# gridap/GridapSolvers.jl

Hardware: AMD Instinct MI355X
Metric: DoFs/sec, CG+GMG V-cycle on 3D Poisson Q1 (higher is better)
Workload: dtype f64; 1 GPU; BASELINE configs[1]: 3D Poisson Q1 128^3 cells, 4-level GMG V-cycle, Richardson(Jacobi,10,2/3) pre=post, dense-inverse coarse solve, CG rtol=1e-06, rhs=u=x1+x2 Dirichlet lift; dofs=2048383, nnz=54439939, levels=4

## Files before the change

### gridapsolvers.jl_amd/csrc/gmg_amd.hip

```cpp
#include "../../include/gmg_amd.h"
#include "kernels.hpp"
#include "comm.hpp"

#include <algorithm>
#include <cmath>
#include <cstdarg>
#include <cstdio>
#include <cstdlib>
#include <cstring>
#include <functional>
#include <map>
#include <memory>
#include <mutex>
#include <exception>
#include <string>
#include <thread>
#include <atomic>
#include <chrono>
#include <unordered_map>
#include <vector>

using namespace gmg;

namespace {
// ... 346 lines not shown
  DevCSR A, P, R;
  double *dinv = nullptr;
  Smoother pre, post;
  Smoother pcorr;
  bool has_pcorr = false;
  HostCSR hG;
  bool hasG = false;
  DevCSR G;
  double *ptmp = nullptr, *pcor = nullptr;
  bool post_shares_pre = true;
  int64_t n = 0;
  int64_t nvec = 0;
  HaloPlan halo;
  bool split = false;
  struct HostXfer { struct ::gmg_solver *solver; int level; } hostctx{nullptr, 0};
  int64_t nbnd = 0;
  int32_t *gh_rows = nullptr;
  int64_t *gh_ptr = nullptr;
  int32_t *gh_col = nullptr;
  double *gh_val = nullptr;
  int32_t *gh_len = nullptr, *gh_scol = nullptr;
  int64_t *gh_soff = nullptr;
  double *gh_sval = nullptr;
  uint8_t *gh_scode = nullptr;
  double *gh_dict = nullptr;
  bool r_split = false;
  GhostFix rfix;
  double *x = nullptr;
  double *rbuf[2] = {nullptr, nullptr};
  double *sbuf[2] = {nullptr, nullptr};
  uint32_t *pflags = nullptr;
  int pf_nwg = 0;
  uint32_t pf_epoch = 1;
  double *dx = nullptr;
  double *rcur = nullptr;
};

struct ConvLog {
  int maxiter = 0;
  double atol = 0, rtol = 0;
  int num_iters = 0;
  std::vector<double> residuals;
  void configure(int mi, double a, double r)
  {
    maxiter = mi; atol = a; rtol = r;
    residuals.assign((size_t)std::max(mi, 0) + 1, 0.0);
  }
  bool finished(int niter, double e_a, double e_r) const
  {
    return (niter >= maxiter) || (e_r < rtol) || (e_a < atol);
  }
  bool init(double r0)
  {
    num_iters = 0;
    std::fill(residuals.begin(), residuals.end(), 0.0);
    residuals[0] = r0;
    return finished(num_iters, r0, 1.0);
  }
  bool update(double r)
  {
    num_iters += 1;
    if ((size_t)num_iters < residuals.size()) residuals[num_iters] = r;
    return finished(num_iters, r, r / residuals[0]);
  }
  int finalize(double r) const
  {
// ... 186 lines not shown
  int sell_un = 6;
  int nt_loads = 1;
  int nt_rowwise = 1;
  int xcd_remap_big = -1;
  int64_t big_rows = 4000000;
  int sell_defer = 1;
  bool big_level(const DevCSR &M) const { return M.nrows > big_rows; }
  int remap_for_big(const DevCSR &M, int rows_per_wg, int nwg) const
  {
    if (xcd_remap_big >= 0) return xcd_remap_big == 1 ? xcd_remap : xcd_remap_big;
    const int64_t want = (2 * std::max<int64_t>(M.band, 1) + rows_per_wg - 1) / rows_per_wg;
    if (want < 2 || want * 8 * 4 > nwg) return 0;
    return (int)want;
  }
  int use_pattern = 1;
  int pat_un = 9;
  int pat_wgs = 2048;
  int pat_rb = 3;
  int use_opattern = 1;
  int pat_batched = 1;
  int pat_nb = 0;
  int pat_small_wpb = 4;
  int pat_small_wpb2 = 2;
  int pat_emit = 1;
  int64_t pat_coded_min_rows = 500000;
  int gj_mfma = 1;
  int pat_tile = 0;
  int64_t pat_tile_rows = 3500000;
  int pat_wide = 1;
  int pat_strict = 1;
  int persist_wpb_min = 1;
  int persist = 1;
  int persist_regs = 1;
  int persist_fenced = 0;
  int persist_max_slices = 0;
  int n_cus = 0;
  uint32_t *d_perr_dev = nullptr;
  uint32_t *h_perr = nullptr, *d_perr = nullptr;
  int pat_bcast = 1;
  int pat_r2 = 1;
  int pat_zwalk = 1;
  int64_t pat_zwalk_wide_rows = 1000000;
  int pat_zwalk_wide = 1;
  int pat_zwalk_mv = 1;
  int pat_fuse2 = 0, pat_fuse2_w = 0, pat_fuse2_t = 0;
  int pat_box = 0, pat_box_t = 0;
  int64_t pat_box_min_rows = 1000000, pat_box_max_rows = 9000000;
  int64_t pat_fuse2_rows = 1000000;
  int pat_zwalk_T = 12;
  int64_t pat_zwalk_rows = 9000000;
  int pat_r2_wgs = 0;
  int pat_r2_occ = 2;
  int pat_r2mv_dot = 1;
  int pat_pair_p = 1;
  int pat_r2mv = 1;
  int64_t pat_r2mv_min = 100000;
  int pat_fma = 0;
  int pat_rsweep = 1;
  int pat_defer = 1;
  int pat_xnext = 1;
  int pat_close = 1;
  bool r0_dead = false;
  int pat_dinv = 1;
  int pat_shared = 1;
  int one_gather_sweep = 1;
  int tile = kTile;
// ... 2092 lines not shown
        if ((++spins & 0x3ff) == 0) {
          const hipError_t q = hipStreamQuery(stream);
          if (q != hipSuccess && q != hipErrorNotReady) HIP_CHECK(q);
          if (q == hipSuccess && __atomic_load_n(seq, __ATOMIC_ACQUIRE) < want &&
              std::chrono::duration<double>(std::chrono::steady_clock::now() - t0).count() > 2.0)
            throw GmgError{GMG_ERR_HIP, "the device never posted the residual norm (host-mapped memory not visible?): set option host_poll = 0"};
        }
      }
      check_persistent();
      return h_mail->value;
    }
    posted = 0;
    HIP_CHECK(hipMemcpyAsync(h_scalars + slot, d_scalars + slot, sizeof(double), hipMemcpyDeviceToHost, stream));
    HIP_CHECK(hipStreamSynchronize(stream));
    check_persistent();
    return h_scalars[slot];
  }
  double dot(int64_t n, const double *a, const double *b)
  {
    dot_async(n, a, b, 0, false, true);
    return fetch_scalar(0);
  }
  double norm(int64_t n, const double *a)
  {
    dot_async(n, a, a, 0, true, true);
    return fetch_scalar(0);
  }

  void build_patch(Level &L, Smoother &S, bool blocks_only = false);
  void build_patch_operator(Level &L, Smoother &S);
  void free_pattern(DevCSR &M);
  void patch_precond(Level &L, Smoother &S, const double *r, double omega, bool relax, double *dx, double *x);

  bool smooth_persistent(int l, const Smoother &S, double *x, const double *r_in, double *r_out, bool x_zero, int niter, bool dry = false, bool close = false)
  {
    Level &L = lev[l];
    const DevCSR &M = L.A;
    if (!persist || (comm.nranks > 1 && L.halo.present && !L.halo.ovl) || niter < 2) return false;
    if (!(M.sell && M.pat && M.pat_shared && !M.pat_coded && M.pat_k == 3 && M.pat_nruns % 3 == 0)) return false;
    const int nu = M.pat_k * M.pat_nruns;
    const size_t lds = (size_t)M.pat_np * nu * 16 + (size_t)M.pat_np * 8 + 16;
    if (lds > 64 * 1024) return false;
    if (n_cus <= 0) {
      hipDeviceProp_t prop;
      HIP_CHECK(hipGetDeviceProperties(&prop, device));
      n_cus = std::max(1, prop.multiProcessorCount);
    }
    const int rows = 65 - M.pat_k;
    const int nsl = (int)((M.nrows + rows - 1) / rows);
    const int cap = persist_max_slices > 0 ? persist_max_slices : n_cus * 16 * 2;
    if (nsl > cap || nsl > n_cus * 16 * 2 || M.nrows >= (int64_t)1 << 30) return false;
    int wpb = std::max(1, std::min(16, persist_wpb_min));
    while (wpb < 16 && (nsl + wpb - 1) / wpb > n_cus) wpb *= 2;
    int ns = (nsl + wpb - 1) / wpb > n_cus ? 2 : 1;
    const int64_t reach = std::max<int64_t>(-(int64_t)M.pat_minoff, (int64_t)M.pat_maxoff + 2);
    int halo = (int)((reach + (int64_t)wpb * ns * rows - 1) / ((int64_t)wpb * ns * rows));
    while (2 * halo + 1 > 64 && wpb < 16) { wpb *= 2; halo = (int)((reach + (int64_t)wpb * ns * rows - 1) / ((int64_t)wpb * ns * rows)); }
    if (2 * halo + 1 > 64) return false;
    const int nwg = (nsl + wpb * ns - 1) / (wpb * ns);
    if (nwg > n_cus) return false;
    if (dry) return true;
    if (!h_perr) {
      HIP_CHECK(hipHostMalloc((void **)&h_perr, 64, hipHostMallocMapped));
      *h_perr = 0;
      HIP_CHECK(hipHostGetDevicePointer((void **)&d_perr, h_perr, 0));
    }
    if (!d_perr_dev) {
      d_perr_dev = dalloc<uint32_t>(16);
      HIP_CHECK(hipMemsetAsync(d_perr_dev, 0, 64, stream));
    }
    if (!L.pflags || L.pf_nwg < nwg) {
      if (L.pflags) { HIP_CHECK(hipStreamSynchronize(stream)); release(L.pflags, (size_t)L.pf_nwg * 16); }
      L.pflags = dalloc<uint32_t>((size_t)nwg * 16);
      HIP_CHECK(hipMemsetAsync(L.pflags, 0, sizeof(uint32_t) * (size_t)nwg * 16, stream));
      L.pf_nwg = nwg; L.pf_epoch = 1;
    }
    if (!h_perr) {
      HIP_CHECK(hipHostMalloc((void **)&h_perr, 64, hipHostMallocMapped));
      *h_perr = 0;
      HIP_CHECK(hipHostGetDevicePointer((void **)&d_perr, h_perr, 0));
    }
    if (!d_perr_dev) {
      d_perr_dev = dalloc<uint32_t>(16);
      HIP_CHECK(hipMemsetAsync(d_perr_dev, 0, 64, stream));
    }
    SellSmoothArgs a;
    std::memset(&a, 0, sizeof(a));
    a.rowpid = M.rowpid; a.tab = M.ptab; a.tab8 = M.ptab8; a.run_off = M.prun; a.np = M.pat_np; a.nruns = M.pat_nruns;
    a.nrows = M.nrows; a.ncols = M.ncols; a.nslices = nsl;
    a.pdinv = pat_dinv ? M.pdinv : nullptr; a.dinv = L.dinv; a.omega = S.omega;
    a.niter = niter; a.x_zero = x_zero ? 1 : 0; a.close = close && niter >= 2 ? 1 : 0;
    a.r_in = r_in; a.r_out = r_out; a.x = x; a.s_a = L.sbuf[0]; a.s_b = L.sbuf[1];
    a.flags = L.pflags; a.epoch = L.pf_epoch; a.err = d_perr; a.err_dev = d_perr_dev; a.halo_wg = halo; a.fenced = persist_fenced;
    L.pf_epoch += (uint32_t)niter;
    const dim3 g(nwg), b(64 * wpb);
    const bool td = a.pdinv != nullptr;
    const bool mk = pat_strict || !M.ptab8;
    const bool prof = (l == prof_level) && prof_used + 2 <= prof_ev.size();
    if (prof) HIP_CHECK(hipEventRecord(prof_ev[prof_used], stream));
    const int nr = persist_regs && smooth_nr_form(ns, mk, M.pat_nruns) ? M.pat_nruns : 0;
    M.note_smooth("sells_smooth_kernel<NS=%d,TD=%d,MK=%d,NR=%d> wgs=%d wpb=%d", ns, td ? 1 : 0, mk ? 1 : 0, nr, nwg, wpb);
#define GMG_SMOOTH_LAUNCH_MK(NSV, TDV, MKV, NRV)                                                               \
    do {                                                                                                         \
      if constexpr (NRV == 0 || smooth_nr_form(NSV, MKV, NRV))                                                   \
        hipLaunchKernelGGL((sells_smooth_kernel<NSV, TDV, MKV, 0, NRV>), g, b, lds, stream, a);                  \
    } while (0)
#define GMG_SMOOTH_LAUNCH_NR(NSV, TDV, NRV)                                                                    \
    do { if (mk) GMG_SMOOTH_LAUNCH_MK(NSV, TDV, true, NRV); else GMG_SMOOTH_LAUNCH_MK(NSV, TDV, false, NRV); } while (0)
#define GMG_SMOOTH_LAUNCH(NSV, TDV)                                                                            \
    do {                                                                                                         \
      if (nr == 9) GMG_SMOOTH_LAUNCH_NR(NSV, TDV, 9);                                                            \
      else if (nr == 3) GMG_SMOOTH_LAUNCH_NR(NSV, TDV, 3);                                                       \
      else GMG_SMOOTH_LAUNCH_NR(NSV, TDV, 0);                                                                    \
    } while (0)
    if (ns == 2) { if (td) GMG_SMOOTH_LAUNCH(2, true); else GMG_SMOOTH_LAUNCH(2, false); }
    else { if (td) GMG_SMOOTH_LAUNCH(1, true); else GMG_SMOOTH_LAUNCH(1, false); }
#undef GMG_SMOOTH_LAUNCH
#undef GMG_SMOOTH_LAUNCH_NR
#undef GMG_SMOOTH_LAUNCH_MK
    HIP_CHECK(hipGetLastError());
    if (prof) {
      HIP_CHECK(hipEventRecord(prof_ev[prof_used + 1], stream));
      prof_w[prof_used / 2] = niter - a.close;
      prof_xm[prof_used / 2] = 0;
      prof_used += 2;
    }
    return true;
// ... 10 lines not shown
    struct Undefer { gmg_solver &S; ~Undefer() { S.defer_out = false; S.pending_out.clear(); } } undefer{*this};
    defer_out = armed;
    pending_out.clear();
    try {
      if (armed && opt_int("GMG_PERSIST_FORCE_TIMEOUT", 0) > 0) {
        options["GMG_PERSIST_FORCE_TIMEOUT"] = opt_int("GMG_PERSIST_FORCE_TIMEOUT", 0) - 1;
        forced = true;
        force_pending = !multi;
      }
      body();
      if (!persist_defer_throw) {
        if (armed) HIP_CHECK(hipStreamSynchronize(stream));
        check_persistent();
      }
    } catch (const GmgError &) {
      persist_defer_throw = false;
      if (!(armed && persist_tripped)) throw;
      again = true;
    }
    if (armed && multi) {
      persist_defer_throw = false;
      HIP_CHECK(hipStreamSynchronize(stream));
      double flag = ((h_perr && *h_perr) || forced) ? 1.0 : 0.0;
      host_allreduce_sum(&flag);
      if (flag > 0.0) {
        if (h_perr) *h_perr = 0;
        persist = 0;
        again = true;
      }
    }
    if (again) {
      persist_tripped = false;
      ++persist_retries;
      HIP_CHECK(hipStreamSynchronize(stream));
      if (inplace) copy(x_user, scratch_vec(6, lev[0].nvec), n);
      pending_out.clear();
      body();
    }
    defer_out = false;
    const std::vector<PendingOut> todo = pending_out;
    pending_out.clear();
    for (const PendingOut &o : todo) out_vec(o.user, o.dev, o.n, o.memspace);
  }
  bool persist_tripped = false;
  bool persist_defer_throw = false;
  int64_t persist_retries = 0;
  void host_allreduce_sum(double *v)
  {
    if (comm.nranks <= 1) return;
    if (comm.kind == COMM_RCCL) {
      double *slot = d_scalars + kScalarSlots - 1;
      HIP_CHECK(hipMemcpyAsync(slot, v, sizeof(double), hipMemcpyHostToDevice, stream));
      const int rc = comm.api.AllReduce(slot, slot, 1, kNcclDouble, kNcclSum, comm.comm, stream);
      REQUIRE(rc == 0, GMG_ERR_COMM, std::string("ncclAllReduce: ") + comm.api.GetErrorString(rc));
      HIP_CHECK(hipMemcpyAsync(v, slot, sizeof(double), hipMemcpyDeviceToHost, stream));
      HIP_CHECK(hipStreamSynchronize(stream));
    } else
      comm.rfn(comm.ctx, v, 1);
  }
  bool force_pending = false;
  void check_persistent()
  {
    if (!((h_perr && *h_perr) || force_pending)) return;
    if (persist_defer_throw) return;
    force_pending = false;
    if (h_perr) *h_perr = 0;
    persist = 0;
    persist_tripped = true;
    throw GmgError{GMG_ERR_STATE, "one-launch smoothing pass: a neighbour wait timed out (its workgroups were not all resident -- is the GPU shared with "
                                  "other persistent kernels?); the results of this call are invalid, the handle now runs with GMG_PERSIST=0"};
  }

  double *smooth(int l, Smoother &S, double *x, const double *r_in, bool x_zero, bool r_dead = false)
  {
    Level &L = lev[l];
    r_dead = r_dead && pat_close && comm.nranks == 1;
    const int64_t n = L.n;
    const bool r_internal = (r_in == L.rbuf[0] || r_in == L.rbuf[1]);
    if (S.niter <= 0) {
      if (x_zero) zero(x, n);
      if (!r_internal) { copy(L.rbuf[0], r_in, n); return L.rbuf[0]; }
      return const_cast<double *>(r_in);
    }
    if (S.kind == SM_JACOBI && one_gather()) {
      const bool ovl = comm.nranks > 1 && L.halo.present && L.halo.ovl;
      const double *cur = r_in;
      double *out = r_internal ? const_cast<double *>(r_in) : L.rbuf[0];
      const int block = ovl ? std::max(1, std::min(L.halo.depth, S.niter)) : S.niter;
      const bool rsw = pat_defer && rsweep_level(L);
      const bool sell64 = L.A.sell && !L.A.pat && !L.A.comp_idx && !L.A.vdict && !L.A.opat;
      const bool defer = (pat_defer && L.A.pat_shared) ||
                         (sell_defer && !(comm.nranks > 1 && L.split) && ((sell64 && sell_un >= 6 && sell_un < 9) || (L.A.sell && L.A.opat && sell_un < 27)));
      for (int done = 0; done < S.niter; done += block) {
        const int nb = std::min(block, S.niter - done);
        const bool first = done == 0;
        if (ovl) {
          if (cur != out) { copy(out, cur, n); cur = out; }
          exchange(l, out);
        }
        const bool xz0 = x_zero && first;
        const bool one_launch = smooth_persistent(l, S, x, cur, out, xz0, nb, true);
        if (rsw && !one_launch) {
          L.s0_ready = false;
          const double *prev = nullptr;
          if (comm.nranks > 1 && L.halo.present && !L.halo.ovl && cur != L.rbuf[0] && cur != L.rbuf[1]) {
            copy(L.rbuf[0], cur, n);
            cur = L.rbuf[0];
          }
          if (pat_fuse2) ensure_z2(L.A);
          const bool fuse2 = fuse2_level(L);
          const bool xnext = pat_xnext && !fuse2 && (nb & 1) == 0 && comm.nranks == 1 && xnext_kernel(L.A);
          L.A.xnext_used = xnext;
          const int nsw = (xnext && r_dead) ? nb - 1 : nb;
          for (int it = 0; it < nsw; ++it) {
            double *next = (cur == L.rbuf[0]) ? L.rbuf[1] : L.rbuf[0];
            if (fuse2 && (it & 1) == 0 && it + 1 < nb) {
              const bool prof = (l == prof_level) && (prof_seq++ % (uint64_t)prof_stride == 0) && prof_used + 2 <= prof_ev.size();
              if (prof) HIP_CHECK(hipEventRecord(prof_ev[prof_used], stream));
              launch_z2sweep(L.A, cur, next, x, xz0 && it == 0, S.omega);
              if (prof) {
                HIP_CHECK(hipEventRecord(prof_ev[prof_used + 1], stream));
                prof_w[prof_used / 2] = 2;
                prof_xm[prof_used / 2] = 2;
                prof_used += 2;
              }
              prev = nullptr;
              cur = next;
              ++it;
              continue;
            }
            int xmode = 0;
            bool xz = xz0 && it == 0;
            if (xnext) xmode = (it & 1) ? 1 : 3;
            else if ((it & 1) == 0 && it + 1 < nb) xmode = 1;
// ... 144 lines not shown
    const int k = std::max(1, std::min(L.halo.depth, S.niter));
    const int last = S.niter - k * ((S.niter - 1) / k);
    return L.ovl_layers - last * L.ovl_sweep_reach >= L.ovl_r_reach;
  }
  void cycle(int l, double *x, const double *r_in, bool x_zero, int ctype)
  {
    if (host_timeline < 0) host_timeline = opt_int("GMG_HOST_TIMELINE", 0);
    Level &L = lev[l];
    if (l == nlev - 1) {
      StepTimer tm(*this, "coarse", l);
      coarse_solve(r_in, x);
      return;
    }
    Level &C = lev[l + 1];
    double *r;
    { StepTimer tm(*this, "pre-smooth", l); r = smooth(l, L.pre, x, r_in, x_zero); }
    const int passes = (ctype == GMG_V_CYCLE) ? 1 : 2;
    for (int pass = 0; pass < passes; ++pass) {
      if (pass == 1) r = smooth(l, L.post, x, r, false);
      const bool ovl_l = comm.nranks > 1 && L.halo.present && L.halo.ovl;
      if (!(ovl_l && skip_r_after(L, pass == 0 ? L.pre : L.post)) && !L.r_split) exchange(l, r);
      if (redist.present && l + 1 == sub_from) {
        const int child = (pass == 0) ? ctype : (ctype == GMG_W_CYCLE ? GMG_W_CYCLE : GMG_V_CYCLE);
        restrict_into(l, r, redist.glue_r);
        redistribute(redist.to_sub, 0, redist.glue_r, C.rbuf[0]);
        if (redist.member) cycle(l + 1, C.x, C.rbuf[0], true, child);
        else shadow_cycle(l + 1, child);
        redistribute(redist.from_sub, 2, C.x, redist.glue_x);
        spmv_addto(L.P, redist.glue_x, L.dx, x);
        apply_A_sub(l, L.dx, r, &L.post);
        continue;
      }
      if (comm.nranks > 1 && l + 1 == rep_from) restrict_replicate(l, r, C.rbuf[0]);
      else if (l + 1 < nlev - 1 && emits_s0(C, C.pre, L.R)) {
        StepTimer tm(*this, "restrict+s0", l);
        spmv_set(L.R, r, C.rbuf[0], C.sbuf[0], C.dinv, C.pre.omega);
        C.s0_ready = true; C.s0_src = C.rbuf[0]; C.s0_omega = C.pre.omega;
      } else {
      StepTimer tm(*this, "restrict", l);
      restrict_into(l, r, C.rbuf[0]);
      }
      const int child = (pass == 0) ? ctype : (ctype == GMG_W_CYCLE ? GMG_W_CYCLE : GMG_V_CYCLE);
      cycle(l + 1, C.x, C.rbuf[0], true, child);
      exchange(l + 1, C.x);
      if (L.has_pcorr) {
        spmv_set(L.P, C.x, L.dx);
        if (L.hasG) { exchange(l, L.dx); spmv_set(L.G, L.dx, L.ptmp); }
        else apply_A_set(l, L.dx, L.ptmp);
        patch_precond(L, L.pcorr, L.ptmp, 1.0, false, L.pcor, nullptr);
        hipLaunchKernelGGL(prolong_correct_kernel, dim3(grid_for(L.n)), dim3(256), 0, stream, L.n, L.pcor, L.dx, x);
        HIP_CHECK(hipGetLastError());
      } else
      { StepTimer tm(*this, "prolong", l); spmv_addto(L.P, C.x, L.dx, x); }
      if (ovl_l && L.ovl_skip_dx && !L.has_pcorr) spmv_sub(L.A, L.dx, r);
      else
      { StepTimer tm(*this, "r -= A dx", l); apply_A_sub(l, L.dx, r, &L.post); }
    }
    const bool r_dead = l > 0 || r0_dead;
    { StepTimer tm(*this, "post-smooth", l); r = smooth(l, L.post, x, r, false, r_dead); }
    L.rcur = r_dead ? nullptr : r;
  }

  double gmg_solve_dev(double *x, const double *b, double known_res0)
  {
    Level &L0 = lev[0];
    const int64_t n = L0.n;
    const double *r_in;
    bool x_zero;
    if (mode == GMG_MODE_PRECONDITIONER) {
      x_zero = true;
      r_in = b;
    } else {
      apply_A_resid(0, x, b, L0.rbuf[0]);
      r_in = L0.rbuf[0];
      x_zero = false;
    }
    double res = known_res0;
    if (!(res >= 0.0)) res = norm(n, r_in);
    bool done = log.init(res);
    if (done && x_zero) zero(x, n);
    const bool single = (log.maxiter == 1);
    const bool fast = single && known_res0 >= 0.0 && (verbose <= 0 || has_outer());
    while (!done) {
      r0_dead = fast && mode == GMG_MODE_PRECONDITIONER;
// ... 412 lines not shown
      int v = 0;
      HIP_CHECK(hipDeviceGetAttribute(&v, hipDeviceAttributeMultiprocessorCount, device));
      n_cus = std::max(1, v);
    }
    pat_bcast = opt_int("GMG_PAT_BCAST", 1);
    red_fused = opt_int("GMG_RED_FUSED", 1);
    pat_r2 = opt_int("GMG_PAT_R2", 1);
    pat_r2_wgs = opt_int("GMG_PAT_R2_WGS", 0);
    pat_r2_occ = opt_int("GMG_PAT_R2_OCC", 2);
    pat_zwalk = opt_int("GMG_PAT_ZWALK", 1);
    pat_zwalk_T = std::max(1, opt_int("GMG_PAT_ZWALK_T", 12));
    pat_zwalk_mv = opt_int("GMG_PAT_ZWALK_MV", 1);
    pat_zwalk_wide = opt_int("GMG_PAT_ZWALK_WIDE", 1);
    pat_zwalk_wide_rows = opt_int("GMG_PAT_ZWALK_WIDE_ROWS", 1000000);
    pat_zwalk_rows = opt_int("GMG_PAT_ZWALK_ROWS", 9000000);
    pat_fuse2 = opt_int("GMG_PAT_FUSE2", 0);
    pat_fuse2_w = opt_int("GMG_PAT_FUSE2_W", 0);
    pat_fuse2_t = opt_int("GMG_PAT_FUSE2_T", 0);
    pat_fuse2_rows = opt_int("GMG_PAT_FUSE2_ROWS", 1000000);
    pat_box = opt_int("GMG_PAT_BOX", 0);
    pat_box_t = opt_int("GMG_PAT_BOX_T", 0);
    pat_box_min_rows = opt_int("GMG_PAT_BOX_MIN_ROWS", 1000000);
    pat_box_max_rows = opt_int("GMG_PAT_BOX_MAX_ROWS", 9000000);
    persist_wpb_min = opt_int("GMG_PERSIST_WPB", 1);
    pat_r2mv = opt_int("GMG_PAT_R2MV", 1);
    pat_pair_p = opt_int("GMG_PAT_PAIR_P", 1);
    pat_r2mv_dot = opt_int("GMG_PAT_R2MV_DOT", 1);
    pat_r2mv_min = opt_int("GMG_PAT_R2MV_MIN", 100000);
    pat_fma = opt_int("GMG_PAT_FMA", 0);
    persist = opt_int("GMG_PERSIST", 1);
    if (comm.kind == COMM_HOST && !opt_int("GMG_PERSIST_SHARED", 0)) persist = 0;
    persist_fenced = opt_int("GMG_PERSIST_FENCED", 0);
    persist_regs = opt_int("GMG_PERSIST_REGS", 1);
    pat_strict = opt_int("GMG_PAT_STRICT", 1);
    pat_wide = opt_int("GMG_PAT_WIDE", 1);
    pat_tile = opt_int("GMG_PAT_TILE", 0);
    pat_tile_rows = opt_int("GMG_PAT_TILE_ROWS", 3500000);
    gj_mfma = opt_int("GMG_GJ_MFMA", 1);
    persist_max_slices = opt_int("GMG_PERSIST_MAX_SLICES", 0);
    pat_coded_min_rows = opt_int("GMG_PAT_CODED_MIN_ROWS", 500000);
    pat_emit = opt_int("GMG_PAT_EMIT", 1);
    pat_small_wpb = std::min(4, std::max(1, opt_int("GMG_PAT_SMALL_WPB", 4)));
    pat_small_wpb2 = std::min(4, std::max(1, opt_int("GMG_PAT_SMALL_WPB2", 2)));
    pat_dinv = opt_int("GMG_PAT_DINV", 1);
    pat_rb = opt_int("GMG_PAT_RB", 3); pat_rb = pat_rb >= 9 ? 9 : (pat_rb <= 1 ? 1 : 3);
    pat_batched = opt_int("GMG_PAT_BATCHED", 1);
    use_opattern = opt_int("GMG_OPATTERN", 1);
    pat_nb = std::min(2, std::max(0, opt_int("GMG_PAT_NB", 0)));
    tile = kTile;
  }
  double *build_inv_diag(const DevCSR &A, int &nzero)
  {
    const int64_t n = A.nrows;
    double *dinv = dalloc<double>((size_t)n);
    if (A.rowptr == nullptr) {
      nzero = 0;
      if (!A.pdinv) { nzero = 1; return dinv; }
      hipLaunchKernelGGL(expand_pattern_dinv_kernel, dim3(grid_for(n)), dim3(256), 0, stream, n, A.rowpid, A.pdinv, dinv);
      HIP_CHECK(hipGetLastError());
      std::vector<double> pd((size_t)A.pat_np);
      HIP_CHECK(hipMemcpyAsync(pd.data(), A.pdinv, sizeof(double) * pd.size(), hipMemcpyDeviceToHost, stream));
      HIP_CHECK(hipStreamSynchronize(stream));
      for (int q = 0; q + 1 < A.pat_np; ++q) if (!std::isfinite(pd[(size_t)q])) nzero++;
      return dinv;
    }
    int *d_nzero = dalloc<int>(1);
// ... 2478 lines not shown
    REQUIRE(h, GMG_ERR_INVALID, "null handle");
    REQUIRE(kind == GMG_COARSE_DENSE_INVERSE || kind == GMG_COARSE_CG_JACOBI || kind == GMG_COARSE_HOST_CALLBACK, GMG_ERR_INVALID,
            "unknown coarse solver kind");
    if (kind == GMG_COARSE_CG_JACOBI) REQUIRE(maxiter >= 0, GMG_ERR_INVALID, "maxiter < 0");
    if (kind == GMG_COARSE_HOST_CALLBACK) REQUIRE(fn, GMG_ERR_INVALID, "null callback");
    h->coarse_kind = kind;
    if (kind == GMG_COARSE_CG_JACOBI) { h->coarse_maxiter = maxiter; h->coarse_atol = atol; h->coarse_rtol = rtol; }
    h->coarse_fn = fn; h->coarse_ctx = ctx;
    h->touch();
  });
}

int gmg_get_coarse_log(gmg_handle_t h, gmg_result *res)
{
  return guarded(h, [&] {
    REQUIRE(h && res, GMG_ERR_INVALID, "null argument");
    REQUIRE(h->coarse_eff == GMG_COARSE_CG_JACOBI && !h->coarse_log.residuals.empty(), GMG_ERR_STATE, "no iterative coarse solve has run");
    h->coarse_log.export_to(res, nullptr, 0, h->coarse_last);
  });
}

namespace {
struct OptionKey { const char *name; bool live; };
const OptionKey kOptionKeys[] = {
  {"GMG_BIG_ROWS", false}, {"GMG_COARSE_HOST_FALLBACK_MAX", false}, {"GMG_COARSE_HOST_MAX", false}, {"GMG_COARSE_AUTO_CG_MIN", false},
  {"GMG_DBG_NOGATHER", false}, {"GMG_EAGER", true}, {"GMG_EAGER_MIN_ROWS", true}, {"GMG_FORCE_PTR64", false}, {"GMG_GJ_MFMA", false}, {"GMG_GJ_WIDE_MIN", false},
  {"GMG_HALO_FUSE_PACK", false}, {"GMG_HALO_FIX_SELL", false}, {"GMG_HALO_FIX_DICT", false}, {"GMG_HALO_SPLIT_R", false}, {"GMG_HOST_ASYNC", false}, {"GMG_IDX16", false}, {"GMG_LANES_LOG2", false}, {"GMG_NT", false},
  {"GMG_NT_ROWWISE", false}, {"GMG_ONE_GATHER", false}, {"GMG_OPATTERN", false}, {"GMG_OVERLAP", false}, {"GMG_PATCH_DEDUP", false},
  {"GMG_PATCH_OPERATOR", false}, {"GMG_PATCH_OP_DEVICE", false}, {"GMG_PATCH_SOURCE_DEDUP", false}, {"GMG_PATTERN", false}, {"GMG_PAT_BATCHED", false},
  {"GMG_PAT_CODED_MIN_ROWS", false}, {"GMG_PAT_DEFER", false}, {"GMG_PAT_DINV", false}, {"GMG_PAT_EMIT", false}, {"GMG_PAT_NB", false},
  {"GMG_PAT_RB", false}, {"GMG_PAT_RSWEEP", false}, {"GMG_PAT_SHARED", false}, {"GMG_PAT_SMALL_WPB", false}, {"GMG_PAT_SMALL_WPB2", false},
  {"GMG_PAT_STRICT", false}, {"GMG_PAT_TILE", false}, {"GMG_PAT_TILE_LDS", false}, {"GMG_PAT_TILE_MIN", false}, {"GMG_PAT_TILE_ROWS", false},
  {"GMG_PAT_TILE_T", false}, {"GMG_PAT_UN", false}, {"GMG_PAT_WGS", false}, {"GMG_PAT_WIDE", false}, {"GMG_PAT_WIDE_LDS", false},
  {"GMG_PAT_WIDE_ROUNDS", false}, {"GMG_PERSIST", false}, {"GMG_PERSIST_FENCED", false}, {"GMG_PERSIST_MAX_SLICES", false}, {"GMG_PERSIST_REGS", false},
  {"GMG_PERSIST_SHARED", false}, {"GMG_PROF_STRIDE", true}, {"GMG_REFRESH", true}, {"GMG_SELL", false}, {"GMG_SELL_BLOCK", false},
  {"GMG_SELL_DEFER", false}, {"GMG_SELL_MAXPAD", false}, {"GMG_SELL_UN", false}, {"GMG_SETUP_TIMING", true}, {"GMG_VDICT", false},
  {"GMG_XCD_REMAP", false}, {"GMG_XCD_REMAP_BIG", false}, {"GMG_X0_ZERO", true}, {"GMG_HOST_POLL", true}, {"GMG_HOST_CHUNK_BYTES", true}, {"GMG_PAT_FMA", false}, {"GMG_PAT_R2", false}, {"GMG_RED_FUSED", false}, {"GMG_GMRES_FUSED", true}, {"GMG_NULLSPACE_FUSED", true}, {"GMG_PAT_R2MV", false}, {"GMG_PAT_R2_OCC", false}, {"GMG_PAT_PAIR_P", false}, {"GMG_PAT_R2MV_DOT", false}, {"GMG_PERSIST_WPB", false}, {"GMG_HOST_TIMELINE", true}, {"GMG_PAT_R2MV_MIN", false}, {"GMG_PAT_BCAST", false}, {"GMG_PAT_R2_WGS", false}, {"GMG_PAT_ZWALK", false}, {"GMG_PAT_ZWALK_T", false}, {"GMG_PAT_ZWALK_ROWS", false}, {"GMG_PAT_ZWALK_MV", false}, {"GMG_PAT_ZWALK_WIDE", false}, {"GMG_PAT_ZWALK_WIDE_ROWS", false}, {"GMG_PAT_FUSE2", false}, {"GMG_PAT_FUSE2_W", false}, {"GMG_PAT_FUSE2_T", false}, {"GMG_PAT_FUSE2_ROWS", false}, {"GMG_PAT_FUSE2_BOX", false}, {"GMG_PAT_BOX", false}, {"GMG_PAT_WIDE_GRID", false}, {"GMG_PAT_BOX_T", false}, {"GMG_PAT_BOX_MIN_ROWS", false}, {"GMG_PAT_BOX_MAX_ROWS", false},
  {"GMG_PERSIST_FORCE_TIMEOUT", true}, {"GMG_PAT_XNEXT", false}, {"GMG_PAT_CLOSE", false}, {"GMG_CG_SPLIT", true},
};
const OptionKey *find_option(const char *key)
{
  if (!key) return nullptr;
  std::string k(key);
  for (auto &c : k) c = (char)std::toupper((unsigned char)c);
  if (k.rfind("GMG_", 0) != 0) k = "GMG_" + k;
  for (const OptionKey &o : kOptionKeys)
    if (k == o.name) return &o;
  return nullptr;
}
}

int gmg_set_option(gmg_handle_t h, const char *key, double value)
{
  return guarded(h, [&] {
    REQUIRE(h, GMG_ERR_INVALID, "null handle");
    const OptionKey *o = find_option(key);
    REQUIRE(o, GMG_ERR_INVALID, std::string("unknown option '") + (key ? key : "(null)") + "' (see the option table in include/gmg_amd.h)");
    auto it = h->options.find(o->name);
    if (it != h->options.end() && it->second == value) return;
    h->options[o->name] = value;
    if (!o->live) h->touch();
  });
}

int gmg_get_option(gmg_handle_t h, const char *key, double *value, int *source)
{
  return guarded(h, [&] {
// ... 868 lines not shown
      total_ms[v] = h->prof_ms_v[v]; launches[v] = h->prof_n_v[v];
      layout_bytes[v] = h->prof_patch ? tmp.layout_bytes : h->sweep_layout_bytes_variant(l, v);
    }
  });
}

int gmg_model_bytes(gmg_handle_t h, double *vcycle_bytes, double *cg_iter_bytes)
{
  return guarded(h, [&] {
    check_ready(h);
    double BV = 0.0;
    for (int l = 0; l < h->nlev - 1; ++l) {
      const Level &L = h->lev[l];
      const double Z = (double)L.A.nnz, N = (double)L.n, ZP = (double)L.P.nnz, NH = (double)h->lev[l + 1].n;
      const double nu2 = (double)(L.pre.niter + L.post.niter);
      BV += nu2 * (12.0 * Z + 68.0 * N) + (12.0 * Z + 28.0 * N) + 24.0 * ZP + 36.0 * N + 28.0 * NH;
    }
    const double NL = (double)h->lev[h->nlev - 1].n;
    BV += 8.0 * NL * NL + 16.0 * NL;
    if (vcycle_bytes) *vcycle_bytes = BV;
    if (cg_iter_bytes) *cg_iter_bytes = BV + 12.0 * (double)h->lev[0].A.nnz + 132.0 * (double)h->lev[0].n;
  });
}

int gmg_sweep_signature(gmg_handle_t h, int lev, char *buf, int cap)
{
  return guarded(h, [&] {
    check_ready(h);
    check_level(h, lev, false);
    REQUIRE(!h->inactive(lev), GMG_ERR_STATE, "this rank holds no part of that level (it lives on a rank subset, gmg_set_redistribution)");
    REQUIRE(buf && cap > 0, GMG_ERR_INVALID, "null buffer");
    const DevCSR &A = h->lev[lev].A;
    const char *sig = A.sweep_sig[0] ? A.sweep_sig : A.op_sig;
    if (A.smooth_sig[0]) std::snprintf(buf, (size_t)cap, "%s%s%s", sig, sig[0] ? " + " : "", A.smooth_sig);
    else std::snprintf(buf, (size_t)cap, "%s", sig);
  });
}

int gmg_level_format(gmg_handle_t h, int lev, int *sell, int *vdict, int *idx16, double *stream_bytes_per_nnz, double *padding)
{
  return guarded(h, [&] {
    check_ready(h);
    check_level(h, lev, false);
    REQUIRE(!h->inactive(lev), GMG_ERR_STATE, "this rank holds no part of that level (it lives on a rank subset, gmg_set_redistribution)");
    const DevCSR &A = h->lev[lev].A;
    if (sell) *sell = A.pat ? 2 : (A.sell ? (A.opat ? 3 : 1) : 0);
    if (vdict) *vdict = A.vdict ? 1 : 0;
    if (idx16) *idx16 = A.comp_idx ? 1 : 0;
    if (stream_bytes_per_nnz) *stream_bytes_per_nnz = (A.sell && (A.pat || A.vdict || A.comp_idx || A.opat)) ? A.stream_bytes_per_nnz : 12.0;
    if (padding) *padding = A.sell && A.nnz > 0 ? (double)A.zpad / (double)A.nnz : 1.0;
  });
}

int gmg_stream_probe(gmg_handle_t h, int64_t nbytes, int reps, double *gbytes_per_s)
{
  return guarded(h, [&] {
    REQUIRE(h && gbytes_per_s, GMG_ERR_INVALID, "null argument");
    REQUIRE(nbytes >= 4096 && reps >= 1, GMG_ERR_INVALID, "bad probe size");
    const int64_t n2 = nbytes / 16;
    double *src = nullptr, *dst = nullptr;
    HIP_CHECK(hipMalloc((void **)&src, (size_t)n2 * 16));
    if (hipMalloc((void **)&dst, (size_t)n2 * 16) != hipSuccess) { (void)hipFree(src); throw GmgError{GMG_ERR_ALLOC, "probe buffers"}; }
    HIP_CHECK(hipMemsetAsync(src, 0, (size_t)n2 * 16, h->stream));
    hipEvent_t e0, e1;
    HIP_CHECK(hipEventCreate(&e0)); HIP_CHECK(hipEventCreate(&e1));
    const int grid = (int)std::min<int64_t>((n2 + 255) / 256, 256 * 32);
    hipLaunchKernelGGL(stream_copy_kernel, dim3(grid), dim3(256), 0, h->stream, n2, src, dst);
// ... 50 lines not shown
```

### gridapsolvers.jl_amd/csrc/kernels.hpp

```cpp
#pragma once
#include <hip/hip_runtime.h>
#include <stdint.h>

namespace gmg {

constexpr int kBlock = 256;
constexpr int kTile = 2048;

enum Epi : int {
  EPI_SET = 0,
  EPI_SUB = 1,
  EPI_RESID = 2,
  EPI_SWEEP = 3,
  EPI_ADDTO = 4
};

__device__ __forceinline__ int remap_block(int b, int nb, int on)
{
  if (!on || nb < 64) return b;
  if (on > 1) {
    const int G = on << 3, g = b / G;
    if ((g + 1) * G > nb) return b;
    const int wi = b - g * G;
    return g * G + (wi & 7) * on + (wi >> 3);
// ... 2735 lines not shown
        const double rn = e0[i] - s;
        const double sk = omega * (du * e0[i]);
        if (XM == 0) a.x2[r] = e2[i] + sk;
        else if (XM == 2) a.x2[r] = (e2[i] + omega * (du * rp[i])) + sk;
        a.y[r] = rn;
      }
    }
  }
}

struct SellSmoothArgs {
  const uint16_t *rowpid;
  const PatEntry *tab;
  const double *tab8;
  const int32_t *run_off;
  int np, nruns;
  int64_t nrows, ncols;
  int nslices;
  const double *pdinv;
  const double *dinv;
  double omega;
  int niter, x_zero;
  const double *r_in;
  double *r_out;
  double *x;
  double *s_a, *s_b;
  uint32_t *flags;
  uint32_t epoch;
  uint32_t *err;
  int halo_wg;
  int fenced;
  uint32_t *err_dev;
  int close;
};

__device__ __forceinline__ double ld_agent(const double *p)
{
  return __longlong_as_double((long long)__hip_atomic_load(reinterpret_cast<const unsigned long long *>(p), __ATOMIC_RELAXED, __HIP_MEMORY_SCOPE_AGENT));
}
__device__ __forceinline__ void st_agent(double *p, double v)
{
  __hip_atomic_store(reinterpret_cast<unsigned long long *>(p), (unsigned long long)__double_as_longlong(v), __ATOMIC_RELAXED, __HIP_MEMORY_SCOPE_AGENT);
}

constexpr bool smooth_nr_form(int ns, bool mk, int nruns) { return (nruns == 9 || nruns == 3) && !(ns == 2 && !mk && nruns == 9); }
template <int NS, bool TD, bool MK, int DBG = 0, int NR = 0>
__global__ __launch_bounds__(1024) void sells_smooth_kernel(SellSmoothArgs a)
{
  constexpr int K = 3, ROWS = 65 - K, RB = 3;
  static_assert(NR == 0 || DBG == 0, "the ablations are those of the runtime-nruns body");
  static_assert(NR == 0 || smooth_nr_form(NS, MK, NR), "see the register table: the launcher keeps NR = 0 there");
  constexpr bool CREG = NR > 0 && NS == 1;
  extern __shared__ double sp_smem[];
  const int nu = NR > 0 ? K * NR : K * a.nruns;
  const int tot = a.np * nu;
  double *s_tab8 = sp_smem;
  uint32_t *s_msk = reinterpret_cast<uint32_t *>(sp_smem + tot);
  double *s_dinv = sp_smem + (MK ? 2 : 1) * (size_t)tot;
  const int lane = threadIdx.x & 63;
  const int wpb = blockDim.x >> 6, wave = threadIdx.x >> 6;
  const int w = blockIdx.x;
  const int last = (int)a.ncols - 1;
  const int lastrow = (int)a.nrows - 1;
  const double omega = a.omega;
  int pid[NS], row[NS];
  bool own[NS];
  double r[NS], xr[NS], so[NS], dv[NS];
#pragma unroll
  for (int i = 0; i < NS; ++i) {
    const int slice = w * (wpb * NS) + i * wpb + wave;
    row[i] = min(slice, a.nslices - 1) * ROWS + lane;
    own[i] = slice < a.nslices && lane < ROWS && row[i] <= lastrow;
    const int rc = min(row[i], lastrow);
    pid[i] = (int)a.rowpid[rc];
    r[i] = a.r_in[rc];
    { const double xl = a.x[rc]; xr[i] = a.x_zero ? 0.0 : xl; }
    so[i] = a.s_a[rc];
    dv[i] = TD ? 0.0 : a.dinv[rc];
  }
  if (MK) { for (int i = threadIdx.x; i < tot; i += blockDim.x) { const PatEntry en = a.tab[i]; s_tab8[i] = en.v; s_msk[i] = en.m; } }
  else { for (int i = threadIdx.x; i < tot; i += blockDim.x) s_tab8[i] = a.tab8[i]; }
  if (TD)
    for (int i = threadIdx.x; i < a.np; i += blockDim.x) s_dinv[i] = a.pdinv[i];
  __syncthreads();
  if (TD) {
#pragma unroll
    for (int i = 0; i < NS; ++i) dv[i] = s_dinv[pid[i]];
  }
  int gi[NR > 0 ? NS : 1][NR > 0 ? NR : 1];
  double cf[CREG ? K * NR : 1];
  if constexpr (NR > 0) {
    int roff[NR];
#pragma unroll
    for (int q = 0; q < NR; ++q) roff[q] = __builtin_amdgcn_readfirstlane(a.run_off[q]);
#pragma unroll
    for (int i = 0; i < NS; ++i) {
#pragma unroll
      for (int q = 0; q < NR; ++q) gi[i][q] = min(max(row[i] + roff[q], 0), last);
    }
    if constexpr (CREG) {
#pragma unroll
      for (int j = 0; j < K * NR; ++j) cf[j] = s_tab8[pid[0] * nu + j];
    }
  }
  const double *sin = a.s_a;
  double *sout = a.s_b;
  const int nb_lo = max(0, w - a.halo_wg), nb_hi = min((int)gridDim.x - 1, w + a.halo_wg);
  const int nk = a.close ? a.niter - 1 : a.niter;
  for (int k = 0; k < nk; ++k) {
    if (k > 0 && !(DBG & 1)) {
      if (wave == 0 && nb_lo + lane <= nb_hi && nb_lo + lane != w) {
        const uint32_t *f = a.flags + (size_t)(nb_lo + lane) * 16;
        const uint32_t want = a.epoch + (uint32_t)k;
        unsigned spins = 0;
        while ((int32_t)(__hip_atomic_load(f, __ATOMIC_RELAXED, __HIP_MEMORY_SCOPE_AGENT) - want) < 0) {
          if (++spins > (1u << 22)) {
            __hip_atomic_store(a.err, 1u, __ATOMIC_RELAXED, __HIP_MEMORY_SCOPE_SYSTEM);
            if (a.err_dev) __hip_atomic_store(a.err_dev, 1u, __ATOMIC_RELAXED, __HIP_MEMORY_SCOPE_AGENT);
            break;
          }
          __builtin_amdgcn_s_sleep(1);
        }
        if (a.fenced) __builtin_amdgcn_fence(__ATOMIC_ACQUIRE, "agent");
      }
      __syncthreads();
    }
    double acc[NS];
    double G[NR > 0 ? NS : 1][NR > 0 ? NR : 1];
    if constexpr (NR > 0) {
#pragma unroll
      for (int i = 0; i < NS; ++i) {
#pragma unroll
        for (int q = 0; q < NR; ++q) G[i][q] = ld_agent(sin + gi[i][q]);
      }
      __builtin_amdgcn_sched_barrier(0);
    }
#pragma unroll
    for (int i = 0; i < NS; ++i) {
      const uint32_t *tm = s_msk + pid[i] * nu;
      const double *tv = s_tab8 + pid[i] * nu;
      double s = 0.0;
      if constexpr (NR > 0) {
#pragma unroll
        for (int q = 0; q < NR; ++q) {
          double c = G[i][q];
#pragma unroll
// ... 29 lines not shown
          }
        }
      }
      if (MK && !(DBG & 8) && !__all(__builtin_isfinite(s))) {
        s = 0.0;
#pragma unroll 1
        for (int r0 = 0; r0 < a.nruns; ++r0) {
          const double *ga = sin + min(max(row[i] + a.run_off[r0], 0), last);
          double c = (DBG & 2) ? *ga : ld_agent(ga);
#pragma unroll
          for (int t = 0; t < K; ++t) {
            if (t > 0) c = wave_shl1(c);
            const int j = r0 * K + t;
            const double g = __hiloint2double(__double2hiint(c) & (int)tm[j], __double2loint(c));
            s = s + tv[j] * g;
          }
        }
      }
      acc[i] = s;
    }
    const bool publish = k + 1 < nk;
#pragma unroll
    for (int i = 0; i < NS; ++i) {
      xr[i] = xr[i] + so[i];
      const double rn = r[i] - acc[i];
      r[i] = rn;
      so[i] = omega * (dv[i] * rn);
      if (publish && own[i]) { if (DBG & 4) sout[row[i]] = so[i]; else st_agent(sout + row[i], so[i]); }
    }
    if (publish && !(DBG & 16)) {
      asm volatile("s_waitcnt vmcnt(0)" ::: "memory");
      __syncthreads();
      if (threadIdx.x == 0) {
        if (a.fenced) __hip_atomic_store(a.flags + (size_t)w * 16, a.epoch + (uint32_t)(k + 1), __ATOMIC_RELEASE, __HIP_MEMORY_SCOPE_AGENT);
        else __hip_atomic_store(a.flags + (size_t)w * 16, a.epoch + (uint32_t)(k + 1), __ATOMIC_RELAXED, __HIP_MEMORY_SCOPE_AGENT);
      }
    }
    const double *t = sin; sin = sout; sout = const_cast<double *>(t);
  }
  if (a.err_dev && __hip_atomic_load(a.err_dev, __ATOMIC_RELAXED, __HIP_MEMORY_SCOPE_AGENT) != 0u) return;
  if (a.close) {
#pragma unroll
    for (int i = 0; i < NS; ++i) {
      if (own[i]) a.x[row[i]] = xr[i] + so[i];
    }
    return;
  }
#pragma unroll
  for (int i = 0; i < NS; ++i) {
    if (own[i]) { a.x[row[i]] = xr[i]; a.r_out[row[i]] = r[i]; }
  }
}

__global__ void slot_count_kernel(int64_t ne, const int32_t *__restrict__ prow, int32_t *__restrict__ cnt)
{
  for (int64_t q = (int64_t)blockIdx.x * blockDim.x + threadIdx.x; q < ne; q += (int64_t)gridDim.x * blockDim.x) atomicAdd(cnt + prow[q], 1);
}
constexpr int kScanItems = 16, kScanBlock = 256, kScanTile = kScanItems * kScanBlock;
__global__ __launch_bounds__(kScanBlock) void scan_local_kernel(int64_t n, const int32_t *__restrict__ in, int32_t *__restrict__ out, int32_t *__restrict__ totals)
{
  __shared__ int32_t sh[kScanBlock];
  const int64_t base = (int64_t)blockIdx.x * kScanTile + (int64_t)threadIdx.x * kScanItems;
  int32_t v[kScanItems], s = 0;
#pragma unroll
  for (int k = 0; k < kScanItems; ++k) { v[k] = base + k < n ? in[base + k] : 0; s += v[k]; }
  sh[threadIdx.x] = s;
  __syncthreads();
  for (int d = 1; d < kScanBlock; d <<= 1) {
// ... 1515 lines not shown
```

Before: 1.198 billion DoFs/s.

## Fold restriction and prolongation into the persistent Jacobi smoother launch

Adds a fold mode to the persistent SELL smoother kernel. The coarse-level pre-smoother can now compute the restricted residual itself, and the fine-level post-smoother can compute the prolongation itself, each as an extra first phase with its own epoch-flag barrier. Transfer operator patterns are staged in LDS alongside the smoother tables. This removes separate restrict/prolong SpMV launches and their intermediate global writes. In exchange it uses more LDS, adds one extra inter-workgroup sync phase, and hard-fails if a folded pass cannot run as one launch.

```diff
diff --git a/gridapsolvers.jl_amd/csrc/gmg_amd.hip b/gridapsolvers.jl_amd/csrc/gmg_amd.hip
--- a/gridapsolvers.jl_amd/csrc/gmg_amd.hip
+++ b/gridapsolvers.jl_amd/csrc/gmg_amd.hip
@@ -402,6 +402,9 @@
   uint32_t *pflags = nullptr;
   int pf_nwg = 0;
   uint32_t pf_epoch = 1;
+  int fold_pending = 0;
+  const double *fold_src = nullptr;
+  int fold_ran = 0;
   double *dx = nullptr;
   double *rcur = nullptr;
 };
@@ -654,6 +657,7 @@
   int persist_wpb_min = 1;
   int persist = 1;
   int persist_regs = 1;
+  int persist_fold = 7;
   int persist_fenced = 0;
   int persist_max_slices = 0;
   int n_cus = 0;
@@ -2812,14 +2816,25 @@
   void free_pattern(DevCSR &M);
   void patch_precond(Level &L, Smoother &S, const double *r, double omega, bool relax, double *dx, double *x);
 
-  bool smooth_persistent(int l, const Smoother &S, double *x, const double *r_in, double *r_out, bool x_zero, int niter, bool dry = false, bool close = false)
+  bool fold_level(int l, const Smoother &S, const DevCSR &T)
+  {
+    if (!persist_fold || comm.nranks != 1 || S.kind != SM_JACOBI || !one_gather() || S.niter < 2) return false;
+    return smooth_persistent(l, S, nullptr, nullptr, nullptr, false, S.niter, true, false, 1, &T, nullptr);
+  }
+  bool smooth_persistent(int l, const Smoother &S, double *x, const double *r_in, double *r_out, bool x_zero, int niter, bool dry = false, bool close = false,
+                         int fold = 0, const DevCSR *T = nullptr, const double *fsrc = nullptr)
   {
     Level &L = lev[l];
     const DevCSR &M = L.A;
     if (!persist || (comm.nranks > 1 && L.halo.present && !L.halo.ovl) || niter < 2) return false;
     if (!(M.sell && M.pat && M.pat_shared && !M.pat_coded && M.pat_k == 3 && M.pat_nruns % 3 == 0)) return false;
     const int nu = M.pat_k * M.pat_nruns;
-    const size_t lds = (size_t)M.pat_np * nu * 16 + (size_t)M.pat_np * 8 + 16;
+    const size_t lds_own = (size_t)M.pat_np * nu * 16 + (size_t)M.pat_np * 8 + 16;
+    size_t lds = lds_own;
+    if (fold) {
+      if (!(T && T->pat && T->sell && T->pat_generic && !T->pat_shared && T->plen && T->ppoff && T->ppval && T->nrows == M.nrows && T->pat_w > 0)) return false;
+      lds += ((size_t)T->pat_np * T->pat_w * 12 + (size_t)T->pat_np * 4 + 7) / 8 * 8;
+    }
     if (lds > 64 * 1024) return false;
     if (n_cus <= 0) {
       hipDeviceProp_t prop;
@@ -2872,7 +2887,12 @@
     a.niter = niter; a.x_zero = x_zero ? 1 : 0; a.close = close && niter >= 2 ? 1 : 0;
     a.r_in = r_in; a.r_out = r_out; a.x = x; a.s_a = L.sbuf[0]; a.s_b = L.sbuf[1];
     a.flags = L.pflags; a.epoch = L.pf_epoch; a.err = d_perr; a.err_dev = d_perr_dev; a.halo_wg = halo; a.fenced = persist_fenced;
-    L.pf_epoch += (uint32_t)niter;
+    if (fold) {
+      a.fold = fold; a.f_rowpid = T->rowpid; a.f_rowbase = T->rowbase; a.f_plen = T->plen; a.f_poff = T->ppoff; a.f_pval = T->ppval;
+      a.f_np = T->pat_np; a.f_W = T->pat_w; a.f_lds = (int)(lds_own / 8); a.f_x = fsrc; a.f_omega = 0.0;
+      L.fold_ran |= fold;
+    }
+    L.pf_epoch += (uint32_t)niter + (fold ? 1u : 0u);
     const dim3 g(nwg), b(64 * wpb);
     const bool td = a.pdinv != nullptr;
     const bool mk = pat_strict || !M.ptab8;
@@ -2949,6 +2969,7 @@
     if (again) {
       persist_tripped = false;
       ++persist_retries;
+      for (Level &Lf : lev) { Lf.fold_pending = 0; Lf.fold_src = nullptr; }
       HIP_CHECK(hipStreamSynchronize(stream));
       if (inplace) copy(x_user, scratch_vec(6, lev[0].nvec), n);
       pending_out.clear();
@@ -2994,6 +3015,11 @@
     r_dead = r_dead && pat_close && comm.nranks == 1;
     const int64_t n = L.n;
     const bool r_internal = (r_in == L.rbuf[0] || r_in == L.rbuf[1]);
+    const int fold = L.fold_pending;
+    const double *fold_src = L.fold_src;
+    L.fold_pending = 0; L.fold_src = nullptr;
+    const DevCSR *fold_T = fold == 1 ? &lev[l - 1].R : fold == 2 ? &L.P : nullptr;
+    REQUIRE(!fold || (S.kind == SM_JACOBI && one_gather() && r_internal && fold_level(l, S, *fold_T)), GMG_ERR_STATE, "a folded transfer met a pass that does not run as one launch");
     if (S.niter <= 0) {
       if (x_zero) zero(x, n);
       if (!r_internal) { copy(L.rbuf[0], r_in, n); return L.rbuf[0]; }
@@ -3016,7 +3042,14 @@
           exchange(l, out);
         }
         const bool xz0 = x_zero && first;
-        const bool one_launch = smooth_persistent(l, S, x, cur, out, xz0, nb, true);
+        const bool one_launch = smooth_persistent(l, S, x, cur, out, xz0, nb, true, false, fold, fold_T, fold_src);
+        if (fold) {
+          L.s0_ready = false;
+          REQUIRE(one_launch && smooth_persistent(l, S, x, cur, out, xz0, nb, false, r_dead, fold, fold_T, fold_src), GMG_ERR_STATE,
+                  "a folded transfer met a pass that does not run as one launch");
+          cur = out;
+          continue;
+        }
         if (rsw && !one_launch) {
           L.s0_ready = false;
           const double *prev = nullptr;
@@ -3227,6 +3260,11 @@
         continue;
       }
       if (comm.nranks > 1 && l + 1 == rep_from) restrict_replicate(l, r, C.rbuf[0]);
+      else if (l + 1 < nlev - 1 && (persist_fold & 1) && !L.r_split && fold_level(l + 1, C.pre, L.R) &&
+               ((persist_fold & 4) || smooth_persistent(l, L.pre, nullptr, nullptr, nullptr, false, L.pre.niter, true))) {
+        C.fold_pending = 1; C.fold_src = r;
+        C.s0_ready = false;
+      }
       else if (l + 1 < nlev - 1 && emits_s0(C, C.pre, L.R)) {
         StepTimer tm(*this, "restrict+s0", l);
         spmv_set(L.R, r, C.rbuf[0], C.sbuf[0], C.dinv, C.pre.omega);
@@ -3245,6 +3283,9 @@
         patch_precond(L, L.pcorr, L.ptmp, 1.0, false, L.pcor, nullptr);
         hipLaunchKernelGGL(prolong_correct_kernel, dim3(grid_for(L.n)), dim3(256), 0, stream, L.n, L.pcor, L.dx, x);
         HIP_CHECK(hipGetLastError());
+      } else if ((persist_fold & 2) && !ovl_l && fold_level(l, L.post, L.P)) {
+        L.fold_pending = 2; L.fold_src = C.x;
+        continue;
       } else
       { StepTimer tm(*this, "prolong", l); spmv_addto(L.P, C.x, L.dx, x); }
       if (ovl_l && L.ovl_skip_dx && !L.has_pcorr) spmv_sub(L.A, L.dx, r);
@@ -3723,6 +3764,7 @@
     if (comm.kind == COMM_HOST && !opt_int("GMG_PERSIST_SHARED", 0)) persist = 0;
     persist_fenced = opt_int("GMG_PERSIST_FENCED", 0);
     persist_regs = opt_int("GMG_PERSIST_REGS", 1);
+    persist_fold = opt_int("GMG_PERSIST_FOLD", 7);
     pat_strict = opt_int("GMG_PAT_STRICT", 1);
     pat_wide = opt_int("GMG_PAT_WIDE", 1);
     pat_tile = opt_int("GMG_PAT_TILE", 0);
@@ -6267,7 +6309,7 @@
   {"GMG_PAT_RB", false}, {"GMG_PAT_RSWEEP", false}, {"GMG_PAT_SHARED", false}, {"GMG_PAT_SMALL_WPB", false}, {"GMG_PAT_SMALL_WPB2", false},
   {"GMG_PAT_STRICT", false}, {"GMG_PAT_TILE", false}, {"GMG_PAT_TILE_LDS", false}, {"GMG_PAT_TILE_MIN", false}, {"GMG_PAT_TILE_ROWS", false},
   {"GMG_PAT_TILE_T", false}, {"GMG_PAT_UN", false}, {"GMG_PAT_WGS", false}, {"GMG_PAT_WIDE", false}, {"GMG_PAT_WIDE_LDS", false},
-  {"GMG_PAT_WIDE_ROUNDS", false}, {"GMG_PERSIST", false}, {"GMG_PERSIST_FENCED", false}, {"GMG_PERSIST_MAX_SLICES", false}, {"GMG_PERSIST_REGS", false},
+  {"GMG_PAT_WIDE_ROUNDS", false}, {"GMG_PERSIST", false}, {"GMG_PERSIST_FENCED", false}, {"GMG_PERSIST_FOLD", false}, {"GMG_PERSIST_MAX_SLICES", false}, {"GMG_PERSIST_REGS", false},
   {"GMG_PERSIST_SHARED", false}, {"GMG_PROF_STRIDE", true}, {"GMG_REFRESH", true}, {"GMG_SELL", false}, {"GMG_SELL_BLOCK", false},
   {"GMG_SELL_DEFER", false}, {"GMG_SELL_MAXPAD", false}, {"GMG_SELL_UN", false}, {"GMG_SETUP_TIMING", true}, {"GMG_VDICT", false},
   {"GMG_XCD_REMAP", false}, {"GMG_XCD_REMAP_BIG", false}, {"GMG_X0_ZERO", true}, {"GMG_HOST_POLL", true}, {"GMG_HOST_CHUNK_BYTES", true}, {"GMG_PAT_FMA", false}, {"GMG_PAT_R2", false}, {"GMG_RED_FUSED", false}, {"GMG_GMRES_FUSED", true}, {"GMG_NULLSPACE_FUSED", true}, {"GMG_PAT_R2MV", false}, {"GMG_PAT_R2_OCC", false}, {"GMG_PAT_PAIR_P", false}, {"GMG_PAT_R2MV_DOT", false}, {"GMG_PERSIST_WPB", false}, {"GMG_HOST_TIMELINE", true}, {"GMG_PAT_R2MV_MIN", false}, {"GMG_PAT_BCAST", false}, {"GMG_PAT_R2_WGS", false}, {"GMG_PAT_ZWALK", false}, {"GMG_PAT_ZWALK_T", false}, {"GMG_PAT_ZWALK_ROWS", false}, {"GMG_PAT_ZWALK_MV", false}, {"GMG_PAT_ZWALK_WIDE", false}, {"GMG_PAT_ZWALK_WIDE_ROWS", false}, {"GMG_PAT_FUSE2", false}, {"GMG_PAT_FUSE2_W", false}, {"GMG_PAT_FUSE2_T", false}, {"GMG_PAT_FUSE2_ROWS", false}, {"GMG_PAT_FUSE2_BOX", false}, {"GMG_PAT_BOX", false}, {"GMG_PAT_WIDE_GRID", false}, {"GMG_PAT_BOX_T", false}, {"GMG_PAT_BOX_MIN_ROWS", false}, {"GMG_PAT_BOX_MAX_ROWS", false},
@@ -7202,7 +7244,8 @@
     REQUIRE(buf && cap > 0, GMG_ERR_INVALID, "null buffer");
     const DevCSR &A = h->lev[lev].A;
     const char *sig = A.sweep_sig[0] ? A.sweep_sig : A.op_sig;
-    if (A.smooth_sig[0]) std::snprintf(buf, (size_t)cap, "%s%s%s", sig, sig[0] ? " + " : "", A.smooth_sig);
+    const int fr = h->lev[lev].fold_ran;
+    if (A.smooth_sig[0]) std::snprintf(buf, (size_t)cap, "%s%s%s folds=%s", sig, sig[0] ? " + " : "", A.smooth_sig, fr == 3 ? "R+P" : fr == 1 ? "R" : fr == 2 ? "P" : "none");
     else std::snprintf(buf, (size_t)cap, "%s", sig);
   });
 }
diff --git a/gridapsolvers.jl_amd/csrc/kernels.hpp b/gridapsolvers.jl_amd/csrc/kernels.hpp
--- a/gridapsolvers.jl_amd/csrc/kernels.hpp
+++ b/gridapsolvers.jl_amd/csrc/kernels.hpp
@@ -2791,6 +2791,16 @@
   int fenced;
   uint32_t *err_dev;
   int close;
+  int fold;
+  const uint16_t *f_rowpid;
+  const int32_t *f_rowbase;
+  const int32_t *f_plen;
+  const int32_t *f_poff;
+  const double *f_pval;
+  int f_np, f_W;
+  int f_lds;
+  const double *f_x;
+  double f_omega;
 };
 
 __device__ __forceinline__ double ld_agent(const double *p)
@@ -2800,6 +2810,25 @@
 __device__ __forceinline__ void st_agent(double *p, double v)
 {
   __hip_atomic_store(reinterpret_cast<unsigned long long *>(p), (unsigned long long)__double_as_longlong(v), __ATOMIC_RELAXED, __HIP_MEMORY_SCOPE_AGENT);
+}
+
+template <int FU>
+__device__ __forceinline__ double fold_row_sum(const double *tv, const int32_t *to, int W, int len, int lmax, uint32_t base8, const double *__restrict__ x)
+{
+  double s = 0.0;
+#pragma unroll 1
+  for (int j = 0; j < lmax; j += FU) {
+    double g[FU];
+#pragma unroll
+    for (int u = 0; u < FU; ++u) g[u] = ld_off(x, base8 + (uint32_t)to[min(j + u, W - 1)]);
+#pragma unroll
+    for (int u = 0; u < FU; ++u) {
+      double gu = g[u], vu = tv[min(j + u, W - 1)];
+      if (!(j + u < len)) { gu = __hiloint2double(0, __double2loint(gu)); vu = 0.0; }
+      s = s + vu * gu;
+    }
+  }
+  return s;
 }
 
 constexpr bool smooth_nr_form(int ns, bool mk, int nruns) { return (nruns == 9 || nruns == 3) && !(ns == 2 && !mk && nruns == 9); }
@@ -2825,6 +2854,8 @@
   int pid[NS], row[NS];
   bool own[NS];
   double r[NS], xr[NS], so[NS], dv[NS];
+  int fpid[NS];
+  uint32_t fbase8[NS];
 #pragma unroll
   for (int i = 0; i < NS; ++i) {
     const int slice = w * (wpb * NS) + i * wpb + wave;
@@ -2832,20 +2863,58 @@
     own[i] = slice < a.nslices && lane < ROWS && row[i] <= lastrow;
     const int rc = min(row[i], lastrow);
     pid[i] = (int)a.rowpid[rc];
-    r[i] = a.r_in[rc];
+    r[i] = 0.0; so[i] = 0.0;
+    if (a.fold != 1) r[i] = a.r_in[rc];
     { const double xl = a.x[rc]; xr[i] = a.x_zero ? 0.0 : xl; }
-    so[i] = a.s_a[rc];
+    if (!a.fold) so[i] = a.s_a[rc];
     dv[i] = TD ? 0.0 : a.dinv[rc];
+    fpid[i] = 0; fbase8[i] = 0u;
+    if (a.fold) { fpid[i] = (int)a.f_rowpid[rc]; fbase8[i] = 8u * (uint32_t)(a.f_rowbase ? a.f_rowbase[rc] : rc); }
   }
   if (MK) { for (int i = threadIdx.x; i < tot; i += blockDim.x) { const PatEntry en = a.tab[i]; s_tab8[i] = en.v; s_msk[i] = en.m; } }
   else { for (int i = threadIdx.x; i < tot; i += blockDim.x) s_tab8[i] = a.tab8[i]; }
   if (TD)
     for (int i = threadIdx.x; i < a.np; i += blockDim.x) s_dinv[i] = a.pdinv[i];
+  if (a.fold) {
+    const int ftot = a.f_np * a.f_W;
+    double *w_val = sp_smem + a.f_lds;
+    int32_t *w_off = reinterpret_cast<int32_t *>(w_val + ftot);
+    int32_t *w_len = w_off + ftot;
+    for (int i = threadIdx.x; i < ftot; i += blockDim.x) { w_val[i] = a.f_pval[i]; w_off[i] = a.f_poff[i]; }
+    for (int i = threadIdx.x; i < a.f_np; i += blockDim.x) w_len[i] = a.f_plen[i];
+  }
   __syncthreads();
   if (TD) {
 #pragma unroll
     for (int i = 0; i < NS; ++i) dv[i] = s_dinv[pid[i]];
   }
+  if (a.fold) {
+    const int W = a.f_W;
+    const double *f_val = sp_smem + a.f_lds;
+    const int32_t *f_off = reinterpret_cast<const int32_t *>(f_val + a.f_np * W);
+    const int32_t *f_len = f_off + a.f_np * W;
+#pragma unroll
+    for (int i = 0; i < NS; ++i) {
+      const int fp = fpid[i];
+      const int len = f_len[fp];
+      int lmax = len;
+#pragma unroll
+      for (int o = 32; o > 0; o >>= 1) lmax = max(lmax, __shfl_xor(lmax, o));
+      lmax = __builtin_amdgcn_readfirstlane(lmax);
+      const double s = lmax > 9 ? fold_row_sum<27>(f_val + fp * W, f_off + fp * W, W, len, lmax, fbase8[i], a.f_x)
+                                : fold_row_sum<9>(f_val + fp * W, f_off + fp * W, W, len, lmax, fbase8[i], a.f_x);
+      if (a.fold == 1) { r[i] = s; so[i] = omega * (dv[i] * s); }
+      else so[i] = a.f_omega != 0.0 ? a.f_omega * s : s;
+      if (own[i]) st_agent(a.s_a + row[i], so[i]);
+    }
+    asm volatile("s_waitcnt vmcnt(0)" ::: "memory");
+    __syncthreads();
+    if (threadIdx.x == 0) {
+      if (a.fenced) __hip_atomic_store(a.flags + (size_t)w * 16, a.epoch + 1u, __ATOMIC_RELEASE, __HIP_MEMORY_SCOPE_AGENT);
+      else __hip_atomic_store(a.flags + (size_t)w * 16, a.epoch + 1u, __ATOMIC_RELAXED, __HIP_MEMORY_SCOPE_AGENT);
+    }
+  }
+  const uint32_t pb = a.fold ? 1u : 0u;
   int gi[NR > 0 ? NS : 1][NR > 0 ? NR : 1];
   double cf[CREG ? K * NR : 1];
   if constexpr (NR > 0) {
@@ -2865,12 +2934,12 @@
   const double *sin = a.s_a;
   double *sout = a.s_b;
   const int nb_lo = max(0, w - a.halo_wg), nb_hi = min((int)gridDim.x - 1, w + a.halo_wg);
-  const int nk = a.close ? a.niter - 1 : a.niter;
+  const int nk = (a.fold == 2 ? a.niter + 1 : a.niter) - (a.close ? 1 : 0);
   for (int k = 0; k < nk; ++k) {
-    if (k > 0 && !(DBG & 1)) {
+    if ((k > 0 || pb) && !(DBG & 1)) {
       if (wave == 0 && nb_lo + lane <= nb_hi && nb_lo + lane != w) {
         const uint32_t *f = a.flags + (size_t)(nb_lo + lane) * 16;
-        const uint32_t want = a.epoch + (uint32_t)k;
+        const uint32_t want = a.epoch + (uint32_t)k + pb;
         unsigned spins = 0;
         while ((int32_t)(__hip_atomic_load(f, __ATOMIC_RELAXED, __HIP_MEMORY_SCOPE_AGENT) - want) < 0) {
           if (++spins > (1u << 22)) {
@@ -2966,8 +3035,8 @@
       asm volatile("s_waitcnt vmcnt(0)" ::: "memory");
       __syncthreads();
       if (threadIdx.x == 0) {
-        if (a.fenced) __hip_atomic_store(a.flags + (size_t)w * 16, a.epoch + (uint32_t)(k + 1), __ATOMIC_RELEASE, __HIP_MEMORY_SCOPE_AGENT);
-        else __hip_atomic_store(a.flags + (size_t)w * 16, a.epoch + (uint32_t)(k + 1), __ATOMIC_RELAXED, __HIP_MEMORY_SCOPE_AGENT);
+        if (a.fenced) __hip_atomic_store(a.flags + (size_t)w * 16, a.epoch + (uint32_t)(k + 1) + pb, __ATOMIC_RELEASE, __HIP_MEMORY_SCOPE_AGENT);
+        else __hip_atomic_store(a.flags + (size_t)w * 16, a.epoch + (uint32_t)(k + 1) + pb, __ATOMIC_RELAXED, __HIP_MEMORY_SCOPE_AGENT);
       }
     }
     const double *t = sin; sin = sout; sout = const_cast<double *>(t);
```

Result: faster. 1.225 billion DoFs/s (median of 6 runs) (+2.2%).
